# tlk00/BitMagic

Measured on AMD Instinct MI355X. Metric: Gbits/s + % HBM roofline, 256-way fused AND+COUNT on 1B-bit vectors, higher is better.
Workload: dtype u64; 1 GPU; aggregator pipeline combine_and_sub counts-only: 256-way AND+COUNT, 256 x 1000000000-bit vectors in total, data set A (common 10% OR noise 10%: no early exit); vectors=256, bits_per_vector=1000000000, density_q16=6554, blocks_per_vector=15259, blocks_per_rank=15259, hbm_resident_bytes=32279432448

## Files before the change

bitmagic_amd/__init__.py:

```python
from __future__ import annotations

import ctypes as C
from typing import Iterable, Sequence

import numpy as np

from . import _ffi
from ._ffi import BmxError, check, lib
from .sharding import shard_range, allreduce_counts

NULL, FULL, BIT, GAP = 0, 1, 2, 3
AND, OR, XOR, SUB = 0, 1, 2, 3
COUNT_AND, COUNT_XOR, COUNT_OR, COUNT_SUB_AB, COUNT_SUB_BA, COUNT_A, COUNT_B = 6, 7, 8, 9, 10, 11, 12
BLOCK_WORDS, BLOCK_BITS = 2048, 65536
opt_none, opt_compress = 0, 3
ID_MAX = 0xFFFFFFFF
ID_MAX64 = 0xFFFFFFFFFFFFFFFF
BM_UNSORTED, BM_SORTED, BM_SORTED_UNIFORM, BM_UNKNOWN = 0, 1, 2, 3

__all__ = ["context", "bvector", "aggregator", "slice_scanner", "rs_index", "rank_compressor", "group", "gbvector", "gaggregator", "gpipeline", "bit_import_u32", "count_and", "count_or",
           "count_xor", "count_sub", "distance_operation", "distance_matrix", "distance_matrix_dev",
           "COUNT_AND", "COUNT_XOR", "COUNT_OR", "COUNT_SUB_AB", "COUNT_SUB_BA", "COUNT_A", "COUNT_B", "BmxError", "simd_version", "device_count", "agg_run_options",
           "agg_opt_only_counts", "agg_opt_bvect_and_counts", "agg_opt_disable_bvects_and_counts",
           "BM_UNSORTED", "BM_SORTED", "BM_SORTED_UNIFORM", "BM_UNKNOWN"]
# ... 634 lines not shown
    def is_complete(self) -> bool:
        return self._h is not None

    def get_bv_count_vector(self) -> np.ndarray:
        return self._counts

    def operand_bytes(self, nb_from: int = 0, nb_to: int = ID_MAX) -> int:
        b = C.c_uint64()
        check(lib().bmx_pipeline_operand_bytes(self.ctx._h, self._h, nb_from, nb_to, C.byref(b)))
        return b.value

    def describe(self, nb_from: int = 0, nb_to: int = ID_MAX) -> str:
        buf = C.create_string_buffer(256)
        check(lib().bmx_pipeline_describe(self.ctx._h, self._h, nb_from, nb_to, buf, 256, None))
        return buf.value.decode()

    def launches(self, nb_from: int = 0, nb_to: int = ID_MAX) -> int:
        buf = C.create_string_buffer(256); n = C.c_uint32()
        check(lib().bmx_pipeline_describe(self.ctx._h, self._h, nb_from, nb_to, buf, 256, C.byref(n)))
        return n.value

    def __del__(self):
        try:
            if self._h and self.ctx._h:
                lib().bmx_pipeline_destroy(self.ctx._h, self._h)
            self._h = None
        except Exception:
            pass


# ... 696 lines not shown
```

bitmagic_amd/_ffi.py:

```python
from __future__ import annotations

import ctypes as C
import os

_HERE = os.path.dirname(os.path.abspath(__file__))
LIB_PATH = os.environ.get("BMX_LIB") or os.path.join(_HERE, "lib", "libbmx.so")

OK, ERR_BADALLOC, ERR_BADARG, ERR_RANGE, ERR_DEVICE = 0, 1, 2, 3, 4


class BmxError(RuntimeError):
    def __init__(self, status: int, msg: str, detail: str):
        super().__init__(f"{msg}" + (f" [{detail}]" if detail else ""))
        self.status = status


_lib = None


def lib() -> C.CDLL:
    global _lib
    if _lib is not None:
        return _lib
    if not os.path.exists(LIB_PATH):
# ... 63 lines not shown
        "bmx_collection_prepare": (i32, [vp, P(vp), C.c_size_t, i32]),
        "bmx_ctx_pack_stats": (i32, [vp, P(u32), P(u64), P(C.c_float)]),
        "bmx_ctx_pack_run_bytes": (i32, [vp, P(u64)]),
        "bmx_pipeline_create": (i32, [vp, P(vp), P(u32), P(vp), P(u32), C.c_size_t, P(vp)]),
        "bmx_pipeline_destroy": (i32, [vp, vp]),
        "bmx_pipeline_set_search_count_limit": (i32, [vp, vp, u64]),
        "bmx_pipeline_last_windows": (i32, [vp, P(u32), P(u32)]),
        "bmx_pipeline_last_window_groups": (i32, [vp, P(u32), u32, P(u32)]),
        "bmx_pipeline_run_counts": (i32, [vp, vp, u32, u32, P(u64)]),
        "bmx_pipeline_run_counts_dev": (i32, [vp, vp, u32, u32, vp]),
        "bmx_pipeline_run_results": (i32, [vp, vp, P(vp), P(u64), vp, P(vp)]),
        "bmx_pipeline_run_results_range": (i32, [vp, vp, u32, u32, P(vp), P(u64), vp, P(vp)]),
        "bmx_pipeline_run_results_hint": (i32, [vp, vp, u64, u64, P(vp), P(u64), vp, P(vp)]),
        "bmx_pipeline_operand_bytes": (i32, [vp, vp, u32, u32, P(u64)]),
        "bmx_pipeline_describe": (i32, [vp, vp, u32, u32, C.c_char_p, C.c_size_t, P(u32)]),
        "bmx_rs_build": (i32, [vp, vp, P(vp)]),
        "bmx_rs_free": (i32, [vp, vp]),
        "bmx_rs_info": (i32, [vp, P(u64), P(i32)]),
        "bmx_rs_select_format": (i32, [vp, P(i32), P(u64)]),
        "bmx_rs_count": (i32, [vp, P(u64)]),
        "bmx_rs_export": (i32, [vp, vp, vp, vp]),
        "bmx_rank_batch": (i32, [vp, vp, vp, vp, C.c_size_t, vp]),
        "bmx_select_batch": (i32, [vp, vp, vp, vp, C.c_size_t, vp, vp]),
        "bmx_rank_batch_dev": (i32, [vp, vp, vp, vp, C.c_size_t, vp]),
        "bmx_select_batch_dev": (i32, [vp, vp, vp, vp, C.c_size_t, vp, vp]),
        "bmx_rank_compress": (i32, [vp, vp, vp, vp, i32, P(vp)]),
        "bmx_rank_decompress": (i32, [vp, vp, vp, vp, i32, P(vp)]),
        "bmx_rank_compress_many": (i32, [vp, vp, vp, P(vp), C.c_size_t, i32, P(vp)]),
        "bmx_rank_decompress_many": (i32, [vp, vp, vp, P(vp), C.c_size_t, i32, P(vp)]),
        "bmx_group_create": (i32, [P(i32), i32, i32, P(vp)]),
# ... 75 lines not shown
```

bitmagic_amd/csrc/bmx.hip:

```cpp
#include "bmx_internal.h"
#ifdef BMX_DIAG
#include "bmx_diag.h"
#endif
#include "bmx_kernels2.h"
#include "bmx_kernels3.h"
#include "bmx_kernels4.h"
#include "bmx_kernels5.h"
#include "bmx_kernels6.h"
#include "bmx_kernels7.h"
#include "bmx_kernels8.h"
#include "bmx_kernels9.h"
#include "bmx_kernels10.h"
#include "bmx_kernels11.h"
#include "bmx_kernels12.h"
#include "bmx_kernels13.h"
#include "bmx_kernels14.h"
#include "bmx_kernels15.h"

#include <algorithm>
#include <atomic>
#include <chrono>
#include <cstdio>
#include <cstdlib>
#include <cstring>
// ... 635 lines not shown
    memcpy(h.data() + goff, &g, sizeof(g));
    int rc;
    if ((rc = dmalloc(ctx, &d_buf.p, h.size())) || (rc = h2d_staged(ctx, d_buf.p, h.data(), h.size()))) { d_buf.reset(); return rc; }
    *d_midx = (const u32*)d_buf.p; *d_groups = (const CollGroup*)((const char*)d_buf.p + goff);
    return BMX_OK;
}

static bool use_split(const bmx_ctx* ctx, const bmx_pipeline* p, u64 nitems)
{
    if (ctx->pipe_split == 0 || !nitems) return false;
    if (ctx->pipe_split == 1) return nitems <= 65535u * 16u;
    return nitems <= 384u && (u64)p->n_ops >= 24ull * p->ngroups;
}
#define SPLIT_WAVES 8

typedef void (*pipe_bits_fn)(const u64*, const u32*, const u32*, u32, u32, u32, u32, int, u64*);

static u32 pipe_window_cap(u32 wg)
{
    u32 wpb = wg / 64u;
    u32 per_cu = wpb >= 7u ? 1u : 12u / wpb;
    return 256u * per_cu * wpb;
}
struct Windows { u32 nwin, per; };
static Windows even_windows(u32 n, u32 cap)
{
    const u32 nwin = (cap && n) ? (n + cap - 1u) / cap : 1u;
    return {nwin, (n + nwin - 1u) / nwin};
}
struct Stretch { u32 per_wave, grid; };
static Stretch even_stretches(u64 n, u32 waves, int wgs)
// ... 21 lines not shown
            static const u32 cand[3] = {640u, 768u, 512u};
            double best = -1.0;
            for (u32 c : cand) {
                u64 cap = pipe_window_cap(c), nwin = (n + cap - 1) / cap, per = (n + nwin - 1) / nwin;
                double fill = (double)per / (double)cap;
                if (fill > best + 0.02) { best = fill; wg = c; }
            }
        }
    }
    if (!ctx->pipe_nt && !ctx->pipe_wg && rows == 8u && wg > 512u) wg = 512u;
    if (ctx->pipe_window < 0 || (ctx->pipe_window == 0 && ngroups > 4u)) window = 0u;
    else if (ctx->pipe_window > 0) window = (u32)ctx->pipe_window;
    else window = (u32)std::max<u64>(pipe_window_cap(wg) / ((u64)ngroups * (8u / rows)), 1u);
}

template <int ROWS>
static pipe_bits_fn pipe_bits_rows(u32 unroll, bool nt, u32 wg)
{
#define B2(U, NT, WG) (pipe_bits_fn)k_pipe_counts_bits2<U, NT, WG, ROWS>
    if (wg == 256 && nt) {
        if (unroll == 4) return B2(4, true, 256);
        if constexpr (ROWS <= 4) { if (unroll == 8) return B2(8, true, 256); }
    }
    if (wg == 256 && !nt && unroll == 4) return B2(4, false, 256);
    if constexpr (ROWS == 8) {
        if (unroll == 4 && nt) switch (wg) { case 384: return B2(4, true, 384); case 512: return B2(4, true, 512);
                                             case 640: return B2(4, true, 640); case 768: return B2(4, true, 768); default: break; }
        if (unroll == 4 && !nt && wg == 512) return B2(4, false, 512);
    }
#ifdef BMX_TUNE
    if constexpr (ROWS == 8) {
        if (nt && unroll == 4) switch (wg) { case 192: return B2(4, true, 192); case 320: return B2(4, true, 320); case 448: return B2(4, true, 448);
                                             case 576: return B2(4, true, 576); default: break; }
        if (nt && unroll == 2) switch (wg) { case 256: return B2(2, true, 256); case 384: return B2(2, true, 384); case 640: return B2(2, true, 640);
                                             case 1024: return B2(2, true, 1024); default: break; }
        if (nt && unroll == 1 && wg == 256) return B2(1, true, 256);
    } else {
        if (nt && wg == 384) {
            if (unroll == 4) return B2(4, true, 384);
            if constexpr (ROWS <= 4) { if (unroll == 8) return B2(8, true, 384); }
            if constexpr (ROWS <= 2) { if (unroll == 16) return B2(16, true, 384); }
        }
        if (nt && wg == 512 && unroll == 4) return B2(4, true, 512);
    }
#endif
#undef B2
    return nullptr;
}
static pipe_bits_fn pipe_bits_kernel(u32 rows, u32 unroll, bool nt, u32 wg)
{
    switch (rows) {
    case 8: return pipe_bits_rows<8>(unroll, nt, wg);
    case 4: return pipe_bits_rows<4>(unroll, nt, wg);
    case 2: return pipe_bits_rows<2>(unroll, nt, wg);
    case 1: return pipe_bits_rows<1>(unroll, nt, wg);
    default: return nullptr;
    }
}

static int ctx_set_tuning(bmx_ctx* ctx, const char* key, int value)
{
    ARGCHK(ctx && key);
    std::string k(key);
    if (k == "pipe_unroll") { ARGCHK(value == 0 || value == 1 || value == 2 || value == 4 || value == 8 || value == 16); ctx->pipe_unroll = value; }
    else if (k == "pipe_rows") { ARGCHK(value == 0 || value == 8 || value == 4 || value == 2 || value == 1); ctx->pipe_rows = value; }
    else if (k == "pipe_nt") ctx->pipe_nt = value != 0;
    else if (k == "pipe_lds") { ARGCHK(value >= 0 && value <= 160 * 1024); ctx->pipe_lds = value; }
    else if (k == "pipe_slots") { ARGCHK(value == 8 || value == 16); ctx->pipe_slots = value; }
    else if (k == "pipe_staged") { ARGCHK(value >= -1 && value <= 1); ctx->pipe_staged = value; }
    else if (k == "pipe_split") { ARGCHK(value >= -1 && value <= 1); ctx->pipe_split = value; }
    else if (k == "pipe_window") { ARGCHK(value >= -1); ctx->pipe_window = value; }
    else if (k == "or_tile") { ARGCHK(value >= 0 && value <= 3); ctx->or_tile = value; }
    else if (k == "or_rows") { ARGCHK(value >= -1 && value <= 1); ctx->or_rows = value; }
    else if (k == "or_depth") { ARGCHK(value == 4 || value == 8); ctx->or_depth = value; }
    else if (k == "direct_cols") { ARGCHK(value >= 0); ctx->direct_cols = value; }
    else if (k == "pair_stream") { ARGCHK(value == -1 || value == 0 || value == 2 || value == 4 || value == 8); ctx->pair_stream = value; }
    else if (k == "pair_wgs") { ARGCHK(value >= 1 && value <= 8); ctx->pair_wgs = value; }
    else if (k == "range_halves") { ARGCHK(value == 0 || value == 1); ctx->range_halves = value; }
    else if (k == "gap_count") { ARGCHK(value >= -1 && value <= 1); ctx->gap_count = value; }
    else if (k == "agg_shape") { ARGCHK(value == 0 || value == 1); ctx->agg_shape = value; }
    else if (k == "and_rows") { ARGCHK(value >= -1 && value <= 1); ctx->and_rows = value; }
    else if (k == "and_rows_wg") { ARGCHK(value == 128 || value == 256 || value == 512); ctx->and_rows_wg = value; }
    else if (k == "and_rows_depth") { ARGCHK(value == 2 || value == 3 || value == 4 || value == 8); ctx->and_rows_depth = value; }
    else if (k == "and_rows_nt") ctx->and_rows_nt = value != 0;
    else if (k == "and_rows_ipw") { ARGCHK(value >= 0 && value <= 64); ctx->and_rows_ipw = value; }
    else if (k == "ff_window") { ARGCHK(value >= -1); ctx->ff_window = value; }
// ... 42 lines not shown
    delete v;
    return rc;
}
int rs_release(bmx_rs* rs)
{
    bmx_ctx* ctx = rs->ctx;
    const int rc = stream_idle(ctx);
    dfree(ctx, rs->d_bcount); dfree(ctx, rs->d_sub); dfree(ctx, rs->d_rcount); dfree(ctx, rs->d_cum); dfree(ctx, rs->d_gidx); dfree(ctx, rs->d_sample); dfree(ctx, rs->d_lines); dfree(ctx, rs->d_dir8); dfree(ctx, rs->d_sdir); dfree(ctx, rs->d_stop); dfree(ctx, rs->d_sel);
    delete rs;
    return rc;
}
int pipeline_release(bmx_pipeline* p)
{
    bmx_ctx* ctx = p->ctx;
    const int rc = stream_idle(ctx);
    dfree(ctx, p->d_dmat); dfree(ctx, p->d_meta); dfree(ctx, (void*)p->d_descs);
    dfree(ctx, (void*)p->d_udesc); dfree(ctx, p->d_unblk); dfree(ctx, p->d_gmask); dfree(ctx, p->d_gskip);
    dfree(ctx, p->cm_buf);
    delete p;
    return rc;
}
int pending_release(bmx_pending* p)
{
    bmx_ctx* ctx = p->ctx;
    if (p->ev) (void)hipEventDestroy(p->ev);
    if (p->slot >= 0) ctx->pend_used[p->slot >> 6] &= ~(1ull << (p->slot & 63));
    dfree(ctx, p->scratch);
    const int rc = p->v ? vec_release(p->v) : BMX_OK;
    delete p;
    return rc;
// ... 4 lines not shown
    if (ctx->stream) (void)hipStreamSynchronize(ctx->stream);
    while (!ctx->colls.empty()) coll_free(ctx, ctx->colls.size() - 1);
    pool_trim(ctx);
    rz_verify(ctx, nullptr);
    if (ctx->rz_hits) fprintf(stderr, "[bmx redzone] context destroyed with %llu damaged allocation(s) found during its life\n", (unsigned long long)ctx->rz_hits);
    for (auto& kv : ctx->pool_live) { auto rz = ctx->rz_live.find(kv.first); (void)hipFree(rz != ctx->rz_live.end() ? rz->second.raw : kv.first); if (rz != ctx->rz_live.end()) ctx->rz_live.erase(rz); }
    ctx->pool_live.clear();
    ensure_release(ctx, &ctx->scratch, &ctx->scratch_bytes);
    ensure_release(ctx, &ctx->aux, &ctx->aux_bytes);
    if (ctx->d_small) (void)hipFree(ctx->d_small);
    if (ctx->d_slots) (void)hipFree(ctx->d_slots);
    if (ctx->d_done) (void)hipFree(ctx->d_done);
    if (ctx->d_slots2) (void)hipFree(ctx->d_slots2);
    if (ctx->d_done2) (void)hipFree(ctx->d_done2);
    if (ctx->d_cursor) (void)hipFree(ctx->d_cursor);
    if (ctx->h_pend) (void)hipHostFree(ctx->h_pend);
    if (ctx->d_zero) (void)hipFree(ctx->d_zero);
    if (ctx->h_small) (void)hipHostFree(ctx->h_small);
    if (ctx->h_stage) (void)hipHostFree(ctx->h_stage);
    if (ctx->ev_stage) (void)hipEventDestroy(ctx->ev_stage);
    if (ctx->ev0) (void)hipEventDestroy(ctx->ev0);
    if (ctx->ev1) (void)hipEventDestroy(ctx->ev1);
    if (ctx->own_stream && ctx->stream) (void)hipStreamDestroy(ctx->stream);
    delete ctx;
}

extern "C" {

const char* bmx_error_msg(int status)
{
// ... 36 lines not shown
    HIPCHK(hipHostMalloc((void**)&ctx->h_stage, STAGE_BYTES));
    HIPCHK(hipEventCreateWithFlags(&ctx->ev_stage, hipEventDisableTiming));
    HIPCHK(hipMalloc((void**)&ctx->d_slots, COUNT_SLOTS * COUNT_SLOT_STRIDE * sizeof(u64)));
    HIPCHK(hipMemsetAsync(ctx->d_slots, 0, COUNT_SLOTS * COUNT_SLOT_STRIDE * sizeof(u64), ctx->stream));
    HIPCHK(hipMalloc((void**)&ctx->d_zero, 256));
    HIPCHK(hipMemsetAsync(ctx->d_zero, 0, 256, ctx->stream));
    HIPCHK(hipMalloc((void**)&ctx->d_done, FOLD_DONE_WORDS * 4));
    HIPCHK(hipMemsetAsync(ctx->d_done, 0, FOLD_DONE_WORDS * 4, ctx->stream));
    HIPCHK(hipMalloc((void**)&ctx->d_slots2, COUNT_SLOTS * COUNT_SLOT_STRIDE * sizeof(u64)));
    HIPCHK(hipMemsetAsync(ctx->d_slots2, 0, COUNT_SLOTS * COUNT_SLOT_STRIDE * sizeof(u64), ctx->stream));
    HIPCHK(hipMalloc((void**)&ctx->d_done2, FOLD_DONE_WORDS * 4));
    HIPCHK(hipMemsetAsync(ctx->d_done2, 0, FOLD_DONE_WORDS * 4, ctx->stream));
    HIPCHK(hipHostMalloc((void**)&ctx->h_pend, PEND_SLOTS * 8 * sizeof(u64)));
    HIPCHK(hipMalloc((void**)&ctx->d_cursor, 64));
    HIPCHK(hipMemsetAsync(ctx->d_cursor, 0, 64, ctx->stream));
    { int v = 0; if (hipDeviceGetAttribute(&v, hipDeviceAttributeMaxSharedMemoryPerBlock, device) == hipSuccess && v > 0) ctx->max_lds_bytes = (uint32_t)v; else (void)hipGetLastError(); }
    { size_t fr = 0, tot = 0; if (hipMemGetInfo(&fr, &tot) == hipSuccess && fr) ctx->pack_cap = (uint64_t)fr / 4; else (void)hipGetLastError(); }
    if (const char* e = getenv("BMX_DEBUG_REDZONE")) ctx->redzone = atoi(e) != 0;
    if (const char* e = getenv("BMX_PACK_MAX_MB")) { long long mb = atoll(e); if (mb >= 0) ctx->pack_cap = (uint64_t)mb << 20; }
    if (const char* e = getenv("BMX_POOL_MAX_MB")) { long long mb = atoll(e); if (mb >= 0) ctx->pool_cap = (uint64_t)mb << 20; }
    static const char* const env_keys[][2] = {
        {"BMX_PIPE_UNROLL", "pipe_unroll"}, {"BMX_PIPE_ROWS", "pipe_rows"}, {"BMX_PIPE_NT", "pipe_nt"},
        {"BMX_PIPE_WG", "pipe_wg"}, {"BMX_PIPE_WINDOW", "pipe_window"}, {"BMX_PIPE_SPLIT", "pipe_split"}, {"BMX_OR_TILE", "or_tile"}, {"BMX_OR_ROWS", "or_rows"}, {"BMX_OR_DEPTH", "or_depth"}, {"BMX_OR_WINDOW", "or_window"}, {"BMX_DIRECT_COLS", "direct_cols"}, {"BMX_FF_WINDOW", "ff_window"}, {"BMX_GAP_COUNT", "gap_count"}, {"BMX_AND_ROWS", "and_rows"}, {"BMX_AGG_SHAPE", "agg_shape"}, {"BMX_AND_ROWS_WG", "and_rows_wg"}, {"BMX_AND_ROWS_DEPTH", "and_rows_depth"}, {"BMX_AND_ROWS_NT", "and_rows_nt"}, {"BMX_AND_ROWS_IPW", "and_rows_ipw"}, {"BMX_RANGE_HALVES", "range_halves"}, {"BMX_PAIR_STREAM", "pair_stream"}, {"BMX_PAIR_WGS", "pair_wgs"}, {"BMX_RS_LANES", "rs_lanes"}, {"BMX_RS_SELECT_TOP", "rs_select_top"}, {"BMX_RS_SELECT_SEL", "rs_select_sel"}, {"BMX_RS_LINES", "rs_lines"}, {"BMX_RS_SELECT_LINES", "rs_select_lines"}, {"BMX_RS_SDIR_SHIFT", "rs_sdir_shift"}, {"BMX_COLL_SHAPE", "coll_shape"}, {"BMX_COLL_WINDOW", "coll_window"}, {"BMX_COLL_SPLIT", "coll_split"}, {"BMX_COLL_BUILD", "coll_build"}, {"BMX_EQ_BIG", "eq_big"}, {"BMX_PAIR_LOOP", "pair_loop"}, {"BMX_PAIR_NT", "pair_nt"}, {"BMX_EQ_BIG_SHAPE", "eq_big_shape"}, {"BMX_OP2_WGS", "op2_wgs"}, {"BMX_OP2_LOOP", "op2_loop"}, {"BMX_OP2_NT", "op2_nt"}, {"BMX_GAP_PACK", "gap_pack"}, {"BMX_COLL_MEMBERS", "coll_members"}, {"BMX_XCD_SWIZZLE", "xcd_swizzle"}, {"BMX_RANKC_PATH", "rankc_path"}};
    for (auto& kv : env_keys)
        if (const char* e = getenv(kv[0])) (void)ctx_set_tuning(ctx.get(), kv[1], atoi(e));
    g_last_error.clear();
    *out = ctx.release();
    return BMX_OK;
ABI_END }

int bmx_ctx_destroy(bmx_ctx* ctx) { ABI_TRY if (ctx) ctx_release(ctx); return BMX_OK; ABI_END }

int bmx_ctx_set_tuning(bmx_ctx* ctx, const char* key, int value) { ABI_TRY return ctx_set_tuning(ctx, key, value); ABI_END }

int bmx_probe_stream_rw(bmx_ctx* ctx, uint64_t bytes, int sets, int wgs_per_cu, int iters, float* ms_per_pass)
{ ABI_TRY
    ARGCHK(ctx && ms_per_pass && bytes >= 8192 && sets >= 1 && sets <= 8 && wgs_per_cu >= 1 && wgs_per_cu <= 8 && iters >= 1);
    int rc = set_dev(ctx); if (rc) return rc;
// ... 1157 lines not shown
    } else if (!p->has_gap) {
        u32 window; pipe_plan(ctx, pl.nitems, ngroups, pl.rows, pl.wg, pl.unroll, window);
        pl.kernel = CK_BITS; pl.parts = 8u / pl.rows; pl.nt = ctx->pipe_nt != 0; pl.lds = (size_t)ctx->pipe_lds;
        pl.win = even_windows(pl.ncols, window);
    } else if (use_and_rows(ctx, p)) {
        pl.kernel = CK_AND_ROWS; pl.ar_wg = (u32)ctx->and_rows_wg; pl.ar_depth = (u32)ctx->and_rows_depth; pl.ar_ipw = ctx->and_rows_ipw > 0 ? (u32)ctx->and_rows_ipw : 1u;
    } else if (use_gapcount(ctx, p)) {
        pl.kernel = CK_GAPCOUNT; pl.lds = (size_t)(16384 * 2 + 2048) * 4;
    } else {
        pl.kernel = CK_GENERAL; pl.unroll = ctx->pipe_unroll == 1 ? 1u : ctx->pipe_unroll == 2 ? 2u : 4u; pl.lds = 4 * 2048 * 4;
        pl.win = even_windows(pl.ncols, ctx->pipe_window > 0 ? (u32)ctx->pipe_window : 0u);
    }
    return pl;
}

static int pipeline_run_counts_impl(bmx_ctx* ctx, bmx_pipeline* p, uint32_t nb_from, uint32_t nb_to, uint64_t* d_counts, bool may_build, const GroupView* gv = nullptr)
{
    ARGCHK(ctx && p && p->ctx == ctx && d_counts);
    int rc = set_dev(ctx); if (rc) return rc;
    if ((rc = pipe_range(p, nb_from, nb_to))) return rc;
    const u32 ngroups = gv ? gv->ngroups : p->ngroups;
    HIPCHK(hipMemsetAsync(d_counts, 0, (size_t)std::max(ngroups, 1u) * 8, ctx->stream));
    if (nb_from == nb_to || !ngroups) return BMX_OK;
    bmx_coll *ca = nullptr, *cs = nullptr;
    if (!p->h_uids.empty() && (rc = pipe_resolve_colls(ctx, p, may_build, &ca, &cs))) return rc;
    const CountsPlan pl = counts_plan(ctx, p, nb_from, nb_to, ngroups, coll_serve(p, ca));
    const u32* row_off = gv ? gv->row_off : p->d_meta; const u32* and_n = gv ? gv->and_n : p->d_meta + p->ngroups; const u32* sub_n = gv ? gv->sub_n : p->d_meta + 2 * p->ngroups;
    const bool items32 = pl.kernel == CK_AND_ROWS || pl.kernel == CK_GAPCOUNT || pl.kernel == CK_GENERAL;
    if (items32 && pl.nitems > 0xFFFFFFF0ull) { g_last_error = "too many (column, group) items in one run"; return BMX_ERR_RANGE; }
    switch (pl.kernel) {
// ... 7 lines not shown
        hipLaunchKernelGGL(fn, dim3(pl.ncols), dim3(pl.slots * 64), pl.lds, ctx->stream,
                           (const u64* const*)p->d_udesc, (const u32*)p->d_unblk, p->nplanes, gv ? gv->gmask : (const u32*)p->d_gmask, gv ? gv->gskip : (const u32*)p->d_gskip,
                           ngroups, nb_from, pl.ncols, ctx->xcd_swz, (u64*)d_counts);
        break;
    }
    case CK_SPLIT: {
        auto fn = k_pipe_split<2, SPLIT_WAVES>;
        HIPCHK(hipFuncSetAttribute(reinterpret_cast<const void*>(fn), hipFuncAttributeMaxDynamicSharedMemorySize, (int)pl.lds));
        hipLaunchKernelGGL(fn, dim3((u32)pl.nitems), dim3(SPLIT_WAVES * 64), pl.lds, ctx->stream,
                           (const u64*)p->d_dmat, row_off, and_n, sub_n, p->col_stride, ngroups, nb_from, nb_to, 0, (u64*)d_counts,
                           0, (uint4*)nullptr, (u64*)nullptr, (BlockStat*)nullptr);
        break;
    }
    case CK_BITS: {
        if (pl.nitems * pl.parts > 0xFFFFFFF0ull) { g_last_error = "too many work items in one run"; return BMX_ERR_RANGE; }
        pipe_bits_fn fn = pipe_bits_kernel(pl.rows, pl.unroll, pl.nt, pl.wg);
        if (!fn) { g_last_error = "this (pipe_rows, pipe_unroll, pipe_nt, pipe_wg) shape is not compiled into the library"; return BMX_ERR_BADARG; }
        const u32 wpb = pl.wg / 64u;
        for (u32 c0 = 0; c0 < pl.ncols; c0 += pl.win.per) {
            u32 nitems = std::min(pl.win.per, pl.ncols - c0) * ngroups * pl.parts;
            hipLaunchKernelGGL(fn, dim3((nitems + wpb - 1) / wpb), dim3(pl.wg), pl.lds, ctx->stream,
                               (const u64*)p->d_dmat, row_off, and_n, p->col_stride, ngroups, nb_from + c0, nitems, ctx->xcd_swz, (u64*)d_counts);
            KCHK();
        }
        return BMX_OK;
    }
    case CK_AND_ROWS:
        hipLaunchKernelGGL(and_rows_kernel<AR_COUNT>(ctx), dim3((u32)((pl.nitems + pl.ar_ipw - 1u) / pl.ar_ipw)), dim3(pl.ar_wg), pl.lds, ctx->stream,
                           (const u64*)p->d_dmat, row_off, and_n, sub_n, p->col_stride, ngroups, nb_from, (u32)pl.nitems, ctx->xcd_swz, (u64*)d_counts,
                           (uint4*)nullptr, (u64*)nullptr, (BlockStat*)nullptr, 0u, 0xFFFFFFFFu, and_rows_diag_bits(), pl.ar_ipw);
        break;
    case CK_GAPCOUNT:
        HIPCHK(hipFuncSetAttribute(reinterpret_cast<const void*>(k_pipe_counts_gapcount<false>), hipFuncAttributeMaxDynamicSharedMemorySize, (int)pl.lds));
        hipLaunchKernelGGL(HIP_KERNEL_NAME(k_pipe_counts_gapcount<false>), dim3((u32)pl.nitems), dim3(1024), pl.lds, ctx->stream,
                           p->d_dmat, row_off, and_n, sub_n, p->col_stride, ngroups, nb_from, (u32)pl.nitems, (u64*)d_counts,
                           (uint4*)nullptr, (u64*)nullptr, (BlockStat*)nullptr, 0u, 0xFFFFFFFFu);
        break;
// ... 43 lines not shown
    return BMX_OK;
ABI_END }

int bmx_pipeline_set_search_count_limit(bmx_ctx* ctx, bmx_pipeline* p, uint64_t limit)
{ ABI_TRY
    ARGCHK(ctx && p && p->ctx == ctx);
    p->search_limit = (limit == 0 || limit == 0xFFFFFFFFull || limit == 0xFFFFFFFFFFFFull) ? ~0ull : limit;
    return BMX_OK;
ABI_END }

int bmx_pipeline_last_windows(const bmx_pipeline* p, uint32_t* launched, uint32_t* planned)
{ ABI_TRY
    ARGCHK(p);
    if (launched) *launched = p->last_windows;
    if (planned) *planned = p->last_windows_planned;
    return BMX_OK;
ABI_END }

}

struct LimitScratch {
    CollPin pin; DevBuf buf; bool have_cg = false, have_masks = false;
    u64 *d_tot = nullptr, *d_cc = nullptr; u32 *d_own = nullptr, *d_masks = nullptr, *d_end = nullptr; CollGroup* d_cg = nullptr;
    explicit LimitScratch(bmx_ctx* ctx) : buf(ctx) {}
};
static int limit_scratch(bmx_ctx* ctx, bmx_pipeline* p, bool may_build, size_t own_words, size_t mask_words, LimitScratch* s)
{
    int rc; const size_t ng = p->ngroups; bmx_coll *ca = nullptr, *cs = nullptr;
    if (!p->h_uids.empty() && (rc = pipe_resolve_colls(ctx, p, may_build, &ca, &cs))) return rc;
    s->pin.pin(ca, cs);
// ... 1956 lines not shown
```

bitmagic_amd/csrc/bmx_device.h:

```cpp
#pragma once
#include <hip/hip_runtime.h>
#include <stdint.h>

typedef uint8_t  u8;
typedef uint16_t u16;
typedef uint32_t u32;
typedef uint64_t u64;

#define GMETA(e) ((u32)((e) >> 48) & 0x1FFFu)
#define GMETA_NONE 0xFFFFFFFFu
#define BMX_DESC_KIND(d) ((u32)((d) & 3ull))
#define BMX_DESC_PTR(d)  ((d) & ~3ull)

typedef u32 u32x4 __attribute__((ext_vector_type(4)));
typedef const __attribute__((address_space(1))) u32x4* gcptr4;
typedef __attribute__((address_space(1))) u32x4* gptr4;
typedef const __attribute__((address_space(1))) u16* gcptr16;

template <int ROWS> struct Part { u32x4 r[ROWS]; };
typedef Part<8> Blk;

__device__ __forceinline__ gcptr4 as_gc4(u64 addr) { return (gcptr4)(uintptr_t)addr; }
__device__ __forceinline__ gcptr4 as_gc4(const void* p) { return (gcptr4)(uintptr_t)p; }
__device__ __forceinline__ gptr4 as_g4(void* p) { return (gptr4)(uintptr_t)p; }
// ... 698 lines not shown
    u32 k = U;
    fetch(0);
    issue(A);
    fetch(k);
    bool zero;
    do {
        issue(B); fetch(k + U);
        bool z1 = consume(A);
        issue(A); fetch(k + 2 * U);
        bool z2 = consume(B);
        zero = z1 | z2;
        k += 2 * U;
    } while (!zero && k < n + U);
    return zero;
}
```

bitmagic_amd/csrc/bmx_internal.h:

```cpp
#pragma once
#include "../../include/bmx.h"
#include <hip/hip_runtime.h>
#include <stdint.h>

#include <map>
#include <memory>
#include <string>
#include <unordered_map>
#include <vector>

typedef uint8_t  u8;
typedef uint16_t u16;
typedef uint32_t u32;
typedef uint64_t u64;

int bmx_fail_hip(hipError_t e, const char* what, const char* file, int line);
void bmx_set_last_error(const char* msg);
#define HIPCHK(call) do { hipError_t e_ = (call); if (e_ != hipSuccess) return bmx_fail_hip(e_, #call, __FILE__, __LINE__); } while (0)
#define ARGCHK(cond) do { if (!(cond)) { bmx_set_last_error("bad argument: " #cond); return BMX_ERR_BADARG; } } while (0)
#define KCHK() HIPCHK(hipGetLastError())
#define PEND_SLOTS 1024
#include <new>
#include <stdexcept>
int bmx_abi_caught(int kind, const char* what);
// ... 28 lines not shown
    struct RzInfo { void* raw; size_t block; size_t bytes; int line; };
    bool redzone = false;
    std::unordered_map<void*, RzInfo> rz_live;
    uint64_t rz_hits = 0; std::string rz_report;
    long long fail_dmalloc_after = -1;
    bool fail_dmalloc_throws = false;
    int pipe_unroll = 0;
    int pipe_rows = 0;
    int pipe_nt = 1;
    int pipe_wg = 0;
    int pipe_window = 0;
    int pipe_staged = -1;
    int pipe_lds = 0;
    int pipe_slots = 16;
    int pipe_split = -1;
    int or_tile = 0;
    int direct_cols = 384;
    int pair_stream = -1;
    int pair_wgs = 1;
    int range_halves = 1;
    int gap_count = -1;
    int agg_shape = 0;
    int and_rows = -1;
    int and_rows_wg = 256;
    int and_rows_ipw = 0;
    int and_rows_nt = 0;
    int and_rows_depth = 3;
    int ff_window = 0;
    int or_window = 0;
    int or_rows = -1;
// ... 134 lines not shown
```

bitmagic_amd/csrc/bmx_kernels.h:

```cpp
#pragma once
#include "bmx_device.h"

#define DESC_MAKE(ptr, kind) ((u64)(uintptr_t)(ptr) | ((u64)(kind) << 62))
#define DESC_K(d) ((u32)((d) >> 62))
#define DESC_P(d) ((d) & 0x0000FFFFFFFFFFFFull)
#define DESC_MAKE_GAP(ptr, len, sbit) (DESC_MAKE(ptr, K_GAP) | ((u64)((((u32)(len)) << 1) | ((u32)(sbit) & 1u)) << 48))
enum { K_NULL = 0, K_FULL = 1, K_BIT = 2, K_GAP = 3 };

#define ROW_EMPTY 1ull
#define ROW_FULL  2ull
#define ROW_ONES  4ull

struct BlockStat { u32 pop; u32 runs; u32 first; u32 kind; };

__global__ __launch_bounds__(256)
void k_generate(u64 seed, u32 vec_id, int with_common, u32 d, u64 nbits, u64* __restrict__ out, u64 nwords64, u64 word0)
{
    u64 i = (u64)blockIdx.x * blockDim.x + threadIdx.x;
    u64 stride = (u64)gridDim.x * blockDim.x;
    for (; i < nwords64; i += stride) {
        u64 w = word0 + i;
        u64 v = gen_word64(seed, vec_id, w, d);
        if (with_common) v |= gen_word64(seed, 0xFFFFFFFFu, w, d);
        u64 bit0 = w * 64u;
// ... 381 lines not shown

    Blk acc;
    blk_fill(acc, ~0u);
    if (pipe_chain<U, true, 0>(acc, pa, nba, lane)) return;
    if (pipe_chain<U, true, 1>(acc, ps, nbs, lane)) return;
    if (nga | ngs) {
        blk_to_lds(acc, lds, lane);
        if (nga && gap_apply_list<GAP_AND>(pa + na - 1u, nga, lds, lane)) return;
        if (ngs && gap_apply_list<GAP_SUB>(ps + ns - 1u, ngs, lds, lane)) return;
        blk_from_lds(acc, lds, lane);
    }
    u32 cnt = wave_sum(blk_lane_popcount(acc));
    if (lane == 0 && cnt) atomicAdd(reinterpret_cast<unsigned long long*>(&counts[g]), (unsigned long long)cnt);
}

template <int U, bool NT, int WG = 256, int ROWS = 8>
__global__ __launch_bounds__(WG)
void k_pipe_counts_bits2(const u64* __restrict__ dmat, const u32* __restrict__ row_off,
                         const u32* __restrict__ and_n, u32 col_stride,
                         u32 ngroups, u32 col_from, u32 nitems, int xcd_swz, u64* __restrict__ counts)
{
    constexpr u32 PARTS = 8 / ROWS;
    u32 lane = lane_id(), wave = threadIdx.x >> 6, wpb = blockDim.x >> 6;
    u32 bid = xcd_swz ? xcd_remap(blockIdx.x, gridDim.x) : blockIdx.x;
    u32 item = uniform32(bid * wpb + wave);
    if (item >= nitems) return;
    u32 part = item % PARTS, cg = item / PARTS;
    u32 c = cg / ngroups, g = cg - c * ngroups;
    const u64* row = dmat + (size_t)(col_from + c) * col_stride + row_off[g];
    u64 hdr = uniform64(row[0]), flags = uniform64(row[1]);
    if (flags & ROW_EMPTY) return;
    if (flags & ROW_FULL) { if (lane == 0) atomicAdd(reinterpret_cast<unsigned long long*>(&counts[g]), (unsigned long long)(65536u / PARTS)); return; }
    u32 nba = (u32)(hdr & 0xFFFFu), nbs = (u32)((hdr >> 32) & 0xFFFFu);
    u32 na = uniform32(and_n[g]);
    const u64* pa = row + 2;
    const u64* ps = pa + na;
    const u32 poff = part * ROWS * 64u;
    Part<ROWS> acc;
#pragma unroll
    for (int i = 0; i < ROWS; ++i) acc.r[i] = (u32x4)(~0u);
    if (pipe_chain<U, NT, 0, ROWS>(acc, pa, nba, lane, poff)) return;
    if (pipe_chain<U, NT, 1, ROWS>(acc, ps, nbs, lane, poff)) return;
    u32 cnt = 0;
#pragma unroll
    for (int i = 0; i < ROWS; ++i) {
        cnt += __popcll(((u64)acc.r[i].y << 32) | acc.r[i].x);
        cnt += __popcll(((u64)acc.r[i].w << 32) | acc.r[i].z);
    }
    cnt = wave_sum(cnt);
    if (lane == 0 && cnt) atomicAdd(reinterpret_cast<unsigned long long*>(&counts[g]), (unsigned long long)cnt);
}

#ifdef BMX_DIAG
template <int AUX>
__global__ __launch_bounds__(256)
void k_diag_stream_read_buf(const uint4* __restrict__ buf, u64 nblocks8k, u32 blocks_per_wave, int pattern, int xcd_swz, u64* __restrict__ sink)
{
    u32 lane = lane_id();
    u32 bid = xcd_swz ? xcd_remap(blockIdx.x, gridDim.x) : blockIdx.x;
    u64 w = (u64)bid * (blockDim.x >> 6) + (threadIdx.x >> 6);
    u64 nwaves = nblocks8k / blocks_per_wave;
    if (w >= nwaves) return;
    u64 b0 = pattern ? w : w * blocks_per_wave;
    u64 step = pattern ? nwaves : 1;
    u32x4 acc = (u32x4)(0u);
// ... 60 lines not shown
```

include/bmx.h:

```cpp
#ifndef BMX_H
#define BMX_H

#include <stddef.h>
#include <stdint.h>

#ifdef __cplusplus
extern "C" {
#endif

#define BMX_OK            0
#define BMX_ERR_BADALLOC  1
#define BMX_ERR_BADARG    2
#define BMX_ERR_RANGE     3
#define BMX_ERR_DEVICE    4

#define BMX_NULL 0
#define BMX_FULL 1
#define BMX_BIT  2
#define BMX_GAP  3

#define BMX_AND 0
#define BMX_OR  1
#define BMX_XOR 2
#define BMX_SUB 3
// ... 133 lines not shown
int bmx_pipeline_last_windows(const bmx_pipeline* p, uint32_t* launched, uint32_t* planned);
int bmx_pipeline_last_window_groups(const bmx_pipeline* p, uint32_t* out, uint32_t cap, uint32_t* n);
int bmx_pipeline_run_counts_dev(bmx_ctx* ctx, bmx_pipeline* p, uint32_t nb_from, uint32_t nb_to,
                                uint64_t* d_counts);
int bmx_pipeline_run_results(bmx_ctx* ctx, bmx_pipeline* p, bmx_vec** results_out, uint64_t* counts_out,
                             const bmx_vec* or_target_in, bmx_vec** or_target_out);
int bmx_pipeline_run_results_range(bmx_ctx* ctx, bmx_pipeline* p, uint32_t nb_from, uint32_t nb_to, bmx_vec** results_out,
                                   uint64_t* counts_out, const bmx_vec* or_target_in, bmx_vec** or_target_out);
int bmx_pipeline_run_results_hint(bmx_ctx* ctx, bmx_pipeline* p, uint64_t from, uint64_t to, bmx_vec** results_out,
                                  uint64_t* counts_out, const bmx_vec* or_target_in, bmx_vec** or_target_out);
int bmx_pipeline_operand_bytes(bmx_ctx* ctx, bmx_pipeline* p, uint32_t nb_from, uint32_t nb_to,
                               uint64_t* bytes);

int bmx_pipeline_describe(bmx_ctx* ctx, bmx_pipeline* p, uint32_t nb_from, uint32_t nb_to, char* buf, size_t buf_len,
                          uint32_t* n_launches);

int bmx_rs_build(bmx_ctx* ctx, const bmx_vec* v, bmx_rs** out);
int bmx_rs_free(bmx_ctx* ctx, bmx_rs* rs);
int bmx_rs_info(const bmx_rs* rs, uint64_t* bytes, int* has_lines);
int bmx_rs_select_format(const bmx_rs* rs, int* offset_bits, uint64_t* bytes);
int bmx_rs_count(const bmx_rs* rs, uint64_t* count);
int bmx_rs_export(bmx_ctx* ctx, const bmx_rs* rs, uint32_t* bcount, uint64_t* sub_count);
int bmx_rank_batch(bmx_ctx* ctx, const bmx_vec* v, const bmx_rs* rs,
                   const uint64_t* n, size_t q, uint64_t* out);
int bmx_select_batch(bmx_ctx* ctx, const bmx_vec* v, const bmx_rs* rs,
                     const uint64_t* rank, size_t q, uint64_t* pos, uint8_t* found);
int bmx_rank_batch_dev(bmx_ctx* ctx, const bmx_vec* v, const bmx_rs* rs,
                       const uint64_t* d_n, size_t q, uint64_t* d_out);
int bmx_select_batch_dev(bmx_ctx* ctx, const bmx_vec* v, const bmx_rs* rs,
                         const uint64_t* d_rank, size_t q, uint64_t* d_pos, uint8_t* d_found);
// ... 87 lines not shown
```

Baseline: 55300 Gbit/s.

## Add adaptive eager-prefix early-exit path to pipeline AND+COUNT kernel

New measurement: 55190 Gbit/s. Within noise of the previous version (-0.2%).

```diff
diff --git a/bitmagic_amd/__init__.py b/bitmagic_amd/__init__.py
--- a/bitmagic_amd/__init__.py
+++ b/bitmagic_amd/__init__.py
@@ -672,6 +672,11 @@
         buf = C.create_string_buffer(256)
         check(lib().bmx_pipeline_describe(self.ctx._h, self._h, nb_from, nb_to, buf, 256, None))
         return buf.value.decode()
+
+    def exit_stat(self) -> int:
+        n = C.c_uint64()
+        check(lib().bmx_pipeline_exit_stat(self.ctx._h, self._h, C.byref(n)))
+        return int(n.value)
 
     def launches(self, nb_from: int = 0, nb_to: int = ID_MAX) -> int:
         buf = C.create_string_buffer(256); n = C.c_uint32()
diff --git a/bitmagic_amd/_ffi.py b/bitmagic_amd/_ffi.py
--- a/bitmagic_amd/_ffi.py
+++ b/bitmagic_amd/_ffi.py
@@ -101,6 +101,7 @@
         "bmx_pipeline_run_results_hint": (i32, [vp, vp, u64, u64, P(vp), P(u64), vp, P(vp)]),
         "bmx_pipeline_operand_bytes": (i32, [vp, vp, u32, u32, P(u64)]),
         "bmx_pipeline_describe": (i32, [vp, vp, u32, u32, C.c_char_p, C.c_size_t, P(u32)]),
+        "bmx_pipeline_exit_stat": (i32, [vp, vp, P(u64)]),
         "bmx_rs_build": (i32, [vp, vp, P(vp)]),
         "bmx_rs_free": (i32, [vp, vp]),
         "bmx_rs_info": (i32, [vp, P(u64), P(i32)]),
diff --git a/bitmagic_amd/csrc/bmx.hip b/bitmagic_amd/csrc/bmx.hip
--- a/bitmagic_amd/csrc/bmx.hip
+++ b/bitmagic_amd/csrc/bmx.hip
@@ -673,7 +673,7 @@
 }
 #define SPLIT_WAVES 8
 
-typedef void (*pipe_bits_fn)(const u64*, const u32*, const u32*, u32, u32, u32, u32, int, u64*);
+typedef void (*pipe_bits_fn)(const u64*, const u32*, const u32*, u32, u32, u32, u32, int, u64*, u32, u64, u64*);
 
 static u32 pipe_window_cap(u32 wg)
 {
@@ -725,10 +725,10 @@
     else window = (u32)std::max<u64>(pipe_window_cap(wg) / ((u64)ngroups * (8u / rows)), 1u);
 }
 
-template <int ROWS>
+template <int ROWS, int E>
 static pipe_bits_fn pipe_bits_rows(u32 unroll, bool nt, u32 wg)
 {
-#define B2(U, NT, WG) (pipe_bits_fn)k_pipe_counts_bits2<U, NT, WG, ROWS>
+#define B2(U, NT, WG) (pipe_bits_fn)k_pipe_counts_bits2<U, NT, WG, ROWS, E>
     if (wg == 256 && nt) {
         if (unroll == 4) return B2(4, true, 256);
         if constexpr (ROWS <= 4) { if (unroll == 8) return B2(8, true, 256); }
@@ -740,7 +740,8 @@
         if (unroll == 4 && !nt && wg == 512) return B2(4, false, 512);
     }
 #ifdef BMX_TUNE
-    if constexpr (ROWS == 8) {
+    if constexpr (E != 0) return nullptr;
+    else if constexpr (ROWS == 8) {
         if (nt && unroll == 4) switch (wg) { case 192: return B2(4, true, 192); case 320: return B2(4, true, 320); case 448: return B2(4, true, 448);
                                              case 576: return B2(4, true, 576); default: break; }
         if (nt && unroll == 2) switch (wg) { case 256: return B2(2, true, 256); case 384: return B2(2, true, 384); case 640: return B2(2, true, 640);
@@ -758,15 +759,20 @@
 #undef B2
     return nullptr;
 }
-static pipe_bits_fn pipe_bits_kernel(u32 rows, u32 unroll, bool nt, u32 wg)
+template <int E>
+static pipe_bits_fn pipe_bits_kernel_e(u32 rows, u32 unroll, bool nt, u32 wg)
 {
     switch (rows) {
-    case 8: return pipe_bits_rows<8>(unroll, nt, wg);
-    case 4: return pipe_bits_rows<4>(unroll, nt, wg);
-    case 2: return pipe_bits_rows<2>(unroll, nt, wg);
-    case 1: return pipe_bits_rows<1>(unroll, nt, wg);
+    case 8: return pipe_bits_rows<8, E>(unroll, nt, wg);
+    case 4: return pipe_bits_rows<4, E>(unroll, nt, wg);
+    case 2: return pipe_bits_rows<2, E>(unroll, nt, wg);
+    case 1: return pipe_bits_rows<1, E>(unroll, nt, wg);
     default: return nullptr;
     }
+}
+static pipe_bits_fn pipe_bits_kernel(u32 rows, u32 unroll, bool nt, u32 wg, bool prefix = false)
+{
+    return prefix ? pipe_bits_kernel_e<PIPE_EAGER_LEN>(rows, unroll, nt, wg) : pipe_bits_kernel_e<0>(rows, unroll, nt, wg);
 }
 
 static int ctx_set_tuning(bmx_ctx* ctx, const char* key, int value)
@@ -781,6 +787,7 @@
     else if (k == "pipe_staged") { ARGCHK(value >= -1 && value <= 1); ctx->pipe_staged = value; }
     else if (k == "pipe_split") { ARGCHK(value >= -1 && value <= 1); ctx->pipe_split = value; }
     else if (k == "pipe_window") { ARGCHK(value >= -1); ctx->pipe_window = value; }
+    else if (k == "pipe_eager") { ARGCHK(value >= -1 && value <= 1); ctx->pipe_eager = value; }
     else if (k == "or_tile") { ARGCHK(value >= 0 && value <= 3); ctx->or_tile = value; }
     else if (k == "or_rows") { ARGCHK(value >= -1 && value <= 1); ctx->or_rows = value; }
     else if (k == "or_depth") { ARGCHK(value == 4 || value == 8); ctx->or_depth = value; }
@@ -853,6 +860,7 @@
 {
     bmx_ctx* ctx = p->ctx;
     const int rc = stream_idle(ctx);
+    if (ctx->exit_pipe == p) ctx->exit_pipe = nullptr;
     dfree(ctx, p->d_dmat); dfree(ctx, p->d_meta); dfree(ctx, (void*)p->d_descs);
     dfree(ctx, (void*)p->d_udesc); dfree(ctx, p->d_unblk); dfree(ctx, p->d_gmask); dfree(ctx, p->d_gskip);
     dfree(ctx, p->cm_buf);
@@ -887,6 +895,7 @@
     if (ctx->d_slots2) (void)hipFree(ctx->d_slots2);
     if (ctx->d_done2) (void)hipFree(ctx->d_done2);
     if (ctx->d_cursor) (void)hipFree(ctx->d_cursor);
+    if (ctx->d_exit) (void)hipFree(ctx->d_exit);
     if (ctx->h_pend) (void)hipHostFree(ctx->h_pend);
     if (ctx->d_zero) (void)hipFree(ctx->d_zero);
     if (ctx->h_small) (void)hipHostFree(ctx->h_small);
@@ -953,6 +962,8 @@
     HIPCHK(hipHostMalloc((void**)&ctx->h_pend, PEND_SLOTS * 8 * sizeof(u64)));
     HIPCHK(hipMalloc((void**)&ctx->d_cursor, 64));
     HIPCHK(hipMemsetAsync(ctx->d_cursor, 0, 64, ctx->stream));
+    HIPCHK(hipMalloc((void**)&ctx->d_exit, 64));
+    HIPCHK(hipMemsetAsync(ctx->d_exit, 0, 64, ctx->stream));
     { int v = 0; if (hipDeviceGetAttribute(&v, hipDeviceAttributeMaxSharedMemoryPerBlock, device) == hipSuccess && v > 0) ctx->max_lds_bytes = (uint32_t)v; else (void)hipGetLastError(); }
     { size_t fr = 0, tot = 0; if (hipMemGetInfo(&fr, &tot) == hipSuccess && fr) ctx->pack_cap = (uint64_t)fr / 4; else (void)hipGetLastError(); }
     if (const char* e = getenv("BMX_DEBUG_REDZONE")) ctx->redzone = atoi(e) != 0;
@@ -960,7 +971,7 @@
     if (const char* e = getenv("BMX_POOL_MAX_MB")) { long long mb = atoll(e); if (mb >= 0) ctx->pool_cap = (uint64_t)mb << 20; }
     static const char* const env_keys[][2] = {
         {"BMX_PIPE_UNROLL", "pipe_unroll"}, {"BMX_PIPE_ROWS", "pipe_rows"}, {"BMX_PIPE_NT", "pipe_nt"},
-        {"BMX_PIPE_WG", "pipe_wg"}, {"BMX_PIPE_WINDOW", "pipe_window"}, {"BMX_PIPE_SPLIT", "pipe_split"}, {"BMX_OR_TILE", "or_tile"}, {"BMX_OR_ROWS", "or_rows"}, {"BMX_OR_DEPTH", "or_depth"}, {"BMX_OR_WINDOW", "or_window"}, {"BMX_DIRECT_COLS", "direct_cols"}, {"BMX_FF_WINDOW", "ff_window"}, {"BMX_GAP_COUNT", "gap_count"}, {"BMX_AND_ROWS", "and_rows"}, {"BMX_AGG_SHAPE", "agg_shape"}, {"BMX_AND_ROWS_WG", "and_rows_wg"}, {"BMX_AND_ROWS_DEPTH", "and_rows_depth"}, {"BMX_AND_ROWS_NT", "and_rows_nt"}, {"BMX_AND_ROWS_IPW", "and_rows_ipw"}, {"BMX_RANGE_HALVES", "range_halves"}, {"BMX_PAIR_STREAM", "pair_stream"}, {"BMX_PAIR_WGS", "pair_wgs"}, {"BMX_RS_LANES", "rs_lanes"}, {"BMX_RS_SELECT_TOP", "rs_select_top"}, {"BMX_RS_SELECT_SEL", "rs_select_sel"}, {"BMX_RS_LINES", "rs_lines"}, {"BMX_RS_SELECT_LINES", "rs_select_lines"}, {"BMX_RS_SDIR_SHIFT", "rs_sdir_shift"}, {"BMX_COLL_SHAPE", "coll_shape"}, {"BMX_COLL_WINDOW", "coll_window"}, {"BMX_COLL_SPLIT", "coll_split"}, {"BMX_COLL_BUILD", "coll_build"}, {"BMX_EQ_BIG", "eq_big"}, {"BMX_PAIR_LOOP", "pair_loop"}, {"BMX_PAIR_NT", "pair_nt"}, {"BMX_EQ_BIG_SHAPE", "eq_big_shape"}, {"BMX_OP2_WGS", "op2_wgs"}, {"BMX_OP2_LOOP", "op2_loop"}, {"BMX_OP2_NT", "op2_nt"}, {"BMX_GAP_PACK", "gap_pack"}, {"BMX_COLL_MEMBERS", "coll_members"}, {"BMX_XCD_SWIZZLE", "xcd_swizzle"}, {"BMX_RANKC_PATH", "rankc_path"}};
+        {"BMX_PIPE_WG", "pipe_wg"}, {"BMX_PIPE_WINDOW", "pipe_window"}, {"BMX_PIPE_EAGER", "pipe_eager"}, {"BMX_PIPE_SPLIT", "pipe_split"}, {"BMX_OR_TILE", "or_tile"}, {"BMX_OR_ROWS", "or_rows"}, {"BMX_OR_DEPTH", "or_depth"}, {"BMX_OR_WINDOW", "or_window"}, {"BMX_DIRECT_COLS", "direct_cols"}, {"BMX_FF_WINDOW", "ff_window"}, {"BMX_GAP_COUNT", "gap_count"}, {"BMX_AND_ROWS", "and_rows"}, {"BMX_AGG_SHAPE", "agg_shape"}, {"BMX_AND_ROWS_WG", "and_rows_wg"}, {"BMX_AND_ROWS_DEPTH", "and_rows_depth"}, {"BMX_AND_ROWS_NT", "and_rows_nt"}, {"BMX_AND_ROWS_IPW", "and_rows_ipw"}, {"BMX_RANGE_HALVES", "range_halves"}, {"BMX_PAIR_STREAM", "pair_stream"}, {"BMX_PAIR_WGS", "pair_wgs"}, {"BMX_RS_LANES", "rs_lanes"}, {"BMX_RS_SELECT_TOP", "rs_select_top"}, {"BMX_RS_SELECT_SEL", "rs_select_sel"}, {"BMX_RS_LINES", "rs_lines"}, {"BMX_RS_SELECT_LINES", "rs_select_lines"}, {"BMX_RS_SDIR_SHIFT", "rs_sdir_shift"}, {"BMX_COLL_SHAPE", "coll_shape"}, {"BMX_COLL_WINDOW", "coll_window"}, {"BMX_COLL_SPLIT", "coll_split"}, {"BMX_COLL_BUILD", "coll_build"}, {"BMX_EQ_BIG", "eq_big"}, {"BMX_PAIR_LOOP", "pair_loop"}, {"BMX_PAIR_NT", "pair_nt"}, {"BMX_EQ_BIG_SHAPE", "eq_big_shape"}, {"BMX_OP2_WGS", "op2_wgs"}, {"BMX_OP2_LOOP", "op2_loop"}, {"BMX_OP2_NT", "op2_nt"}, {"BMX_GAP_PACK", "gap_pack"}, {"BMX_COLL_MEMBERS", "coll_members"}, {"BMX_XCD_SWIZZLE", "xcd_swizzle"}, {"BMX_RANKC_PATH", "rankc_path"}};
     for (auto& kv : env_keys)
         if (const char* e = getenv(kv[0])) (void)ctx_set_tuning(ctx.get(), kv[1], atoi(e));
     g_last_error.clear();
@@ -2148,6 +2159,12 @@
     return pl;
 }
 
+static bool pipe_eager_run(const bmx_ctx* ctx, const bmx_pipeline* p, const CountsPlan& pl)
+{
+    if (ctx->pipe_eager == 0 || !p->has_bit || 2u * pl.unroll < (u32)PIPE_EAGER_LEN) return false;
+    return ctx->pipe_eager == 1 || pl.win.nwin >= 2u;
+}
+
 static int pipeline_run_counts_impl(bmx_ctx* ctx, bmx_pipeline* p, uint32_t nb_from, uint32_t nb_to, uint64_t* d_counts, bool may_build, const GroupView* gv = nullptr)
 {
     ARGCHK(ctx && p && p->ctx == ctx && d_counts);
@@ -2185,13 +2202,25 @@
     }
     case CK_BITS: {
         if (pl.nitems * pl.parts > 0xFFFFFFF0ull) { g_last_error = "too many work items in one run"; return BMX_ERR_RANGE; }
-        pipe_bits_fn fn = pipe_bits_kernel(pl.rows, pl.unroll, pl.nt, pl.wg);
-        if (!fn) { g_last_error = "this (pipe_rows, pipe_unroll, pipe_nt, pipe_wg) shape is not compiled into the library"; return BMX_ERR_BADARG; }
+        bool prefix = pipe_eager_run(ctx, p, pl);
+        pipe_bits_fn fn = pipe_bits_kernel(pl.rows, pl.unroll, pl.nt, pl.wg, prefix);
+        if (!fn && prefix && ctx->pipe_eager < 0) { prefix = false; fn = pipe_bits_kernel(pl.rows, pl.unroll, pl.nt, pl.wg); }
+        if (!fn) { g_last_error = "this (pipe_rows, pipe_unroll, pipe_nt, pipe_wg, pipe_eager) shape is not compiled into the library"; return BMX_ERR_BADARG; }
+        ctx->exit_counted = prefix; ctx->exit_pipe = p;
+        if (prefix) HIPCHK(hipMemsetAsync(ctx->d_exit, 0, 8, ctx->stream));
         const u32 wpb = pl.wg / 64u;
+        u64 need = 0;
         for (u32 c0 = 0; c0 < pl.ncols; c0 += pl.win.per) {
             u32 nitems = std::min(pl.win.per, pl.ncols - c0) * ngroups * pl.parts;
+            if (!c0) {
+                u64 sampled = 0;
+                for (u64 i0 = 0; i0 < nitems; i0 += (u64)wpb * PIPE_EAGER_SAMPLE) sampled += std::min<u64>(wpb, nitems - i0);
+                need = (sampled + 1u) / 2u;
+            }
+            const u32 eager = !prefix ? PIPE_EAGER_OFF : ctx->pipe_eager == 1 ? (!c0 ? PIPE_EAGER_COUNT_ALL : PIPE_EAGER_ON) : (!c0 ? PIPE_EAGER_COUNT : PIPE_EAGER_ASK);
             hipLaunchKernelGGL(fn, dim3((nitems + wpb - 1) / wpb), dim3(pl.wg), pl.lds, ctx->stream,
-                               (const u64*)p->d_dmat, row_off, and_n, p->col_stride, ngroups, nb_from + c0, nitems, ctx->xcd_swz, (u64*)d_counts);
+                               (const u64*)p->d_dmat, row_off, and_n, p->col_stride, ngroups, nb_from + c0, nitems, ctx->xcd_swz, (u64*)d_counts,
+                               eager, need, ctx->d_exit);
             KCHK();
         }
         return BMX_OK;
@@ -2265,6 +2294,18 @@
     ARGCHK(p);
     if (launched) *launched = p->last_windows;
     if (planned) *planned = p->last_windows_planned;
+    return BMX_OK;
+ABI_END }
+
+int bmx_pipeline_exit_stat(bmx_ctx* ctx, bmx_pipeline* p, uint64_t* n)
+{ ABI_TRY
+    ARGCHK(ctx && p && p->ctx == ctx && n);
+    *n = 0;
+    if (!ctx->exit_counted || ctx->exit_pipe != p) return BMX_OK;
+    int rc = set_dev(ctx); if (rc) return rc;
+    HIPCHK(hipMemcpyAsync(ctx->h_small + 61, ctx->d_exit, 8, hipMemcpyDeviceToHost, ctx->stream));
+    HIPCHK(hipStreamSynchronize(ctx->stream));
+    *n = ctx->h_small[61];
     return BMX_OK;
 ABI_END }
 
diff --git a/bitmagic_amd/csrc/bmx_device.h b/bitmagic_amd/csrc/bmx_device.h
--- a/bitmagic_amd/csrc/bmx_device.h
+++ b/bitmagic_amd/csrc/bmx_device.h
@@ -736,3 +736,24 @@
     } while (!zero && k < n + U);
     return zero;
 }
+
+template <int E, bool NT, int ROWS>
+__device__ __forceinline__ bool pipe_prefix(Part<ROWS>& acc, const u64* __restrict__ plist, u32 n, u32 lane, u32 poff)
+{
+    u64 p[E];
+#pragma unroll
+    for (int e = 0; e < E; ++e) p[e] = plist[(u32)e < n ? (u32)e : n - 1u];
+    Part<ROWS> buf;
+    part_load<ROWS, NT>(buf, as_gc4(uniform64(p[0])) + poff, lane);
+#pragma unroll
+    for (int e = 0; e < E; ++e) {
+#pragma unroll
+        for (int i = 0; i < ROWS; ++i) acc.r[i] &= buf.r[i];
+        if (e + 1 < E) {
+            u64 q = uniform64(p[e + 1]);
+            asm volatile("" : "+s"(q), "+v"(acc.r[ROWS - 1].w));
+            part_load<ROWS, NT>(buf, as_gc4(q) + poff, lane);
+        }
+    }
+    return part_is_zero<ROWS>(acc);
+}
diff --git a/bitmagic_amd/csrc/bmx_internal.h b/bitmagic_amd/csrc/bmx_internal.h
--- a/bitmagic_amd/csrc/bmx_internal.h
+++ b/bitmagic_amd/csrc/bmx_internal.h
@@ -66,6 +66,9 @@
     int pipe_lds = 0;
     int pipe_slots = 16;
     int pipe_split = -1;
+    int pipe_eager = -1;
+    u64* d_exit = nullptr;
+    bool exit_counted = false; const void* exit_pipe = nullptr;
     int or_tile = 0;
     int direct_cols = 384;
     int pair_stream = -1;
diff --git a/bitmagic_amd/csrc/bmx_kernels.h b/bitmagic_amd/csrc/bmx_kernels.h
--- a/bitmagic_amd/csrc/bmx_kernels.h
+++ b/bitmagic_amd/csrc/bmx_kernels.h
@@ -419,11 +419,16 @@
     if (lane == 0 && cnt) atomicAdd(reinterpret_cast<unsigned long long*>(&counts[g]), (unsigned long long)cnt);
 }
 
-template <int U, bool NT, int WG = 256, int ROWS = 8>
+enum { PIPE_EAGER_OFF = 0, PIPE_EAGER_ON = 1, PIPE_EAGER_COUNT = 2, PIPE_EAGER_ASK = 3, PIPE_EAGER_COUNT_ALL = 4 };
+#define PIPE_EAGER_SAMPLE 32u
+#define PIPE_EAGER_LEN 6
+
+template <int U, bool NT, int WG = 256, int ROWS = 8, int E = 0>
 __global__ __launch_bounds__(WG)
 void k_pipe_counts_bits2(const u64* __restrict__ dmat, const u32* __restrict__ row_off,
                          const u32* __restrict__ and_n, u32 col_stride,
-                         u32 ngroups, u32 col_from, u32 nitems, int xcd_swz, u64* __restrict__ counts)
+                         u32 ngroups, u32 col_from, u32 nitems, int xcd_swz, u64* __restrict__ counts,
+                         u32 eager, u64 exit_need, u64* exit_stat)
 {
     constexpr u32 PARTS = 8 / ROWS;
     u32 lane = lane_id(), wave = threadIdx.x >> 6, wpb = blockDim.x >> 6;
@@ -444,16 +449,38 @@
     Part<ROWS> acc;
 #pragma unroll
     for (int i = 0; i < ROWS; ++i) acc.r[i] = (u32x4)(~0u);
-    if (pipe_chain<U, NT, 0, ROWS>(acc, pa, nba, lane, poff)) return;
-    if (pipe_chain<U, NT, 1, ROWS>(acc, ps, nbs, lane, poff)) return;
-    u32 cnt = 0;
-#pragma unroll
-    for (int i = 0; i < ROWS; ++i) {
-        cnt += __popcll(((u64)acc.r[i].y << 32) | acc.r[i].x);
-        cnt += __popcll(((u64)acc.r[i].w << 32) | acc.r[i].z);
-    }
-    cnt = wave_sum(cnt);
-    if (lane == 0 && cnt) atomicAdd(reinterpret_cast<unsigned long long*>(&counts[g]), (unsigned long long)cnt);
+    auto count = [&]() {
+        u32 cnt = 0;
+#pragma unroll
+        for (int i = 0; i < ROWS; ++i) {
+            cnt += __popcll(((u64)acc.r[i].y << 32) | acc.r[i].x);
+            cnt += __popcll(((u64)acc.r[i].w << 32) | acc.r[i].z);
+        }
+        cnt = wave_sum(cnt);
+        if (lane == 0 && cnt) atomicAdd(reinterpret_cast<unsigned long long*>(&counts[g]), (unsigned long long)cnt);
+    };
+    if constexpr (E > 0) {
+        bool pre = eager != PIPE_EAGER_OFF && nba != 0u;
+        if (eager == PIPE_EAGER_COUNT) pre = pre && (bid & (PIPE_EAGER_SAMPLE - 1u)) == 0u;
+        if (pre && eager == PIPE_EAGER_ASK) pre = uniform64(*exit_stat) >= exit_need;
+        if (__builtin_expect(!pre, 1)) {
+            if (pipe_chain<U, NT, 0, ROWS>(acc, pa, nba, lane, poff)) return;
+            if (pipe_chain<U, NT, 1, ROWS>(acc, ps, nbs, lane, poff)) return;
+            count();
+            return;
+        }
+        if (pipe_prefix<E, NT, ROWS>(acc, pa, nba, lane, poff)) {
+            if ((eager == PIPE_EAGER_COUNT || eager == PIPE_EAGER_COUNT_ALL) && lane == 0) atomicAdd(reinterpret_cast<unsigned long long*>(exit_stat), 1ull);
+            return;
+        }
+        if (nba > (u32)E && pipe_chain<1, NT, 0, ROWS>(acc, pa + E, nba - (u32)E, lane, poff)) return;
+        if (pipe_chain<1, NT, 1, ROWS>(acc, ps, nbs, lane, poff)) return;
+        count();
+    } else {
+        if (pipe_chain<U, NT, 0, ROWS>(acc, pa, nba, lane, poff)) return;
+        if (pipe_chain<U, NT, 1, ROWS>(acc, ps, nbs, lane, poff)) return;
+        count();
+    }
 }
 
 #ifdef BMX_DIAG
diff --git a/include/bmx.h b/include/bmx.h
--- a/include/bmx.h
+++ b/include/bmx.h
@@ -171,6 +171,7 @@
 
 int bmx_pipeline_describe(bmx_ctx* ctx, bmx_pipeline* p, uint32_t nb_from, uint32_t nb_to, char* buf, size_t buf_len,
                           uint32_t* n_launches);
+int bmx_pipeline_exit_stat(bmx_ctx* ctx, bmx_pipeline* p, uint64_t* n);
 
 int bmx_rs_build(bmx_ctx* ctx, const bmx_vec* v, bmx_rs** out);
 int bmx_rs_free(bmx_ctx* ctx, bmx_rs* rs);
```
